# peabody124/PosePipeline

Measured on AMD Instinct MI355X. Metric: frames/sec (whole node), detect->2D->3D cascade on 1080p; MPJPE vs reference, higher is better.
Workload: dtype f32; eligible float32 convolutions are evaluated as 2-term float16 splits (22 significand bits under per-channel / per-sample power-of-two scales, 3 products per term) on the 16-bit matrix cores with float32 accumulation (float32-accurate at any input magnitude, not bit-identical: tests/test_gpu_spl

## Files before the change

posepipeline_amd/csrc/api_core.hip:

```cpp
#include <dlfcn.h>

#include <algorithm>
#include <memory>

#include "pp_internal.h"
#include "pp_amax.h"

#include <atomic>
extern std::atomic<int> g_decode_generic, g_split_gemm_epi;

static thread_local std::string g_last_error;

void pp_set_error(const char* fmt, ...) {
    char buf[1024];
    va_list ap;
    va_start(ap, fmt);
    vsnprintf(buf, sizeof(buf), fmt, ap);
    va_end(ap);
    g_last_error = buf;
}

namespace {
struct Roctx {
    int (*push)(const char*) = nullptr;
    int (*pop)() = nullptr;
    Roctx() {
        for (const char* lib : {"librocprofiler-sdk-roctx.so", "librocprofiler-sdk-roctx.so.1", "libroctx64.so", "libroctx64.so.4"}) {
            void* h = dlopen(lib, RTLD_LAZY | RTLD_LOCAL);
            if (!h) continue;
            push = reinterpret_cast<int (*)(const char*)>(dlsym(h, "roctxRangePushA"));
            pop = reinterpret_cast<int (*)()>(dlsym(h, "roctxRangePop"));
            if (push && pop) return;
            push = nullptr; pop = nullptr;
        }
    }
};
const Roctx& roctx() {
    static const Roctx r;
    return r;
}
}

void pp_range_push(const char* name) {
    if (roctx().push) (void)roctx().push(name);
}
void pp_range_pop() {
    if (roctx().pop) (void)roctx().pop();
}

int pp_ctx::ensure_scratch(size_t bytes) {
    if (bytes <= scratch_bytes) return PP_OK;
    if (scratch) {
        PP_HIP_CHECK(hipStreamSynchronize(stream));
        PP_HIP_CHECK(hipFree(scratch));
        scratch = nullptr;
        scratch_bytes = 0;
    }
    size_t want = std::max(bytes, size_t(1) << 20);
    PP_HIP_CHECK(hipMalloc(&scratch, want));
    scratch_bytes = want;
    return PP_OK;
}

extern "C" {

int pp_abi_version(void) { return PP_ABI_VERSION; }

int pp_debug_knob(const char* name, int value) {
    PP_REQUIRE(name && value >= -1 && value <= 1, "pp_debug_knob: name and a value in {-1, 0, 1}");
    if (!strcmp(name, "decode_generic")) g_decode_generic.store(value, std::memory_order_relaxed);
    else if (!strcmp(name, "split_gemm_epilogue")) g_split_gemm_epi.store(value, std::memory_order_relaxed);
    else {
        pp_set_error("pp_debug_knob: unknown knob '%s' (decode_generic, split_gemm_epilogue)", name);
        return PP_ERR_ARG;
    }
    return PP_OK;
}

const char* pp_last_error(void) { return g_last_error.c_str(); }

int pp_device_count(void) {
    int n = 0;
    if (hipGetDeviceCount(&n) != hipSuccess) {
        (void)hipGetLastError();
        return 0;
    }
    return n;
}

int pp_ctx_create(int device, pp_ctx** out) {
    PP_REQUIRE(out != nullptr, "pp_ctx_create: out is NULL");
    *out = nullptr;
    int n = 0;
    hipError_t e = hipGetDeviceCount(&n);
    if (e != hipSuccess || n <= 0) {
        (void)hipGetLastError();
        pp_set_error("pp_ctx_create: no HIP device visible (%s) -- this library has no CPU fallback",
                     e == hipSuccess ? "device count 0" : hipGetErrorString(e));
        return PP_ERR_HIP;
    }
    PP_REQUIRE(device >= 0 && device < n, "pp_ctx_create: device %d out of range [0,%d)", device, n);
    PP_HIP_CHECK(hipSetDevice(device));
    std::unique_ptr<pp_ctx> c(new pp_ctx());
    c->device = device;
    PP_HIP_CHECK(hipStreamCreateWithFlags(&c->stream, hipStreamNonBlocking));
    PP_HIP_CHECK(hipEventCreate(&c->ev_start));
// ... 143 lines not shown

struct pp_net {
    pp_ctx* ctx = nullptr;
    std::vector<pp_op> ops;
    std::vector<pp_buf> bufs;
    std::vector<size_t> buf_off;
    std::vector<size_t> buf_elems;
    float* weights = nullptr;
    size_t n_weights = 0;
    unsigned char* wsplit = nullptr;
    std::vector<long long> wsplit_off;
    int numerics = PP_NET_NUMERICS_EXACT;
    int split_f16 = 0;
    unsigned* amax = nullptr;
    std::vector<int> op_x_slot, op_y_slot, op_post_slot, slot_owner;
    std::vector<int> slot_first, slot_last;
    struct ExtAmax { int buf, slot, first_reader, last_reader; bool provided; };
    std::vector<ExtAmax> ext;
    float* arena = nullptr;
    size_t arena_floats = 0;
    int max_batch = 0;
    hipGraphExec_t graph_exec = nullptr;
    int graph_batch = 0;
    bool use_lanes = true;
    std::vector<hipStream_t> lanes;
    std::vector<int> op_lane;
    std::vector<std::vector<int>> op_waits;
    std::vector<char> op_needs_event;
    std::vector<hipEvent_t> op_done;
    hipEvent_t fork_ev = nullptr;
    std::vector<hipEvent_t> join_ev;
    std::vector<pp_vit_encoder*> vits;
    std::vector<pp_deconv_bf16*> deconvs;

    float* buf_ptr(int b) const { return arena + buf_off[b]; }
    unsigned* amax_slot(int slot) const { return slot >= 0 ? amax + (size_t)slot * max_batch : nullptr; }
};

static ConvArgs net_conv_args(pp_net* net, const pp_op& op, int batch);
static int net_make_lanes(pp_net* net, int n_lanes);

static void net_plan_amax(pp_net* net) {
    const int n = (int)net->ops.size(), nb = (int)net->bufs.size();
    net->op_x_slot.assign(n, -1);
    net->op_y_slot.assign(n, -1);
    net->op_post_slot.assign(n, -1);
    net->slot_owner.clear();
    net->ext.clear();
    if (net->numerics != PP_NET_NUMERICS_SPLIT || !net->split_f16) return;
    auto is_h = [&](int i) { return net->ops[i].type == PP_OP_CONV && net->wsplit_off[i] >= 0; };
    auto tracks = [&](int i) {
        const pp_op& op = net->ops[i];
        if (op.type == PP_OP_UPSAMPLE_ADD) return true;
        return op.type == PP_OP_CONV && pp_conv_tracks_amax(net_conv_args(net, op, 1), is_h(i));
    };
    {
        std::vector<char> written(nb, 0);
        for (int i = 0; i < n; ++i) {
            const pp_op& op = net->ops[i];
            if (is_h(i) && !written[op.in]) {
                pp_net::ExtAmax* e = nullptr;
                for (auto& x : net->ext)
                    if (x.buf == op.in) e = &x;
                if (!e) {
                    net->ext.push_back({op.in, (int)net->slot_owner.size(), i, i, false});
                    net->slot_owner.push_back(-1);
// ... 44 lines not shown
            for (int p : t.producers) net->op_y_slot[p] = t.slot;
        else
            net->op_post_slot[t.producers.back()] = t.slot;
    }
    for (const auto& r : readers) net->op_x_slot[r.first] = tensors[r.second].slot;
}

static int net_reset_amax(pp_net* net, int first, int last, int batch, hipStream_t s) {
    if (!net->amax) return PP_OK;
    int s0 = -1, s1 = -1;
    for (int k = 0; k < (int)net->slot_first.size(); ++k) {
        const int a = net->slot_first[k], b = net->slot_last[k];
        if (a < 0 || b < first || a >= last) continue;
        PP_REQUIRE(a >= first && b < last, "pp_net_run: op range [%d, %d) splits the producers (ops %d .. %d) of a tensor whose per-sample maxima are tracked",
                   first, last, a, b);
    }
    for (int k = 0; k < (int)net->slot_owner.size(); ++k)
        if (net->slot_owner[k] >= first && net->slot_owner[k] < last) {
            if (s0 < 0) s0 = k;
            s1 = k + 1;
        }
    if (s0 >= 0) PP_HIP_CHECK(hipMemsetAsync(net->amax_slot(s0), 0, (size_t)(s1 - s0) * net->max_batch * sizeof(unsigned), s));
    for (auto& e : net->ext) {
        if (e.last_reader < first || e.first_reader >= last) continue;
        if (e.provided) {
            e.provided = false;
            continue;
        }
        PP_HIP_CHECK(hipMemsetAsync(net->amax_slot(e.slot), 0, (size_t)batch * sizeof(unsigned), s));
        int rc = pp_launch_amax(net->buf_ptr(e.buf), batch, net->buf_elems[e.buf], net->amax_slot(e.slot), s);
        if (rc != PP_OK) return rc;
    }
    return PP_OK;
}

static void net_plan_lanes(pp_net* net, int n_lanes) {
    const int n = (int)net->ops.size(), nb = (int)net->bufs.size();
    net->op_lane.assign(n, 0);
    net->op_waits.assign(n, {});
    net->op_needs_event.assign(n, 0);
    std::vector<int> last_writer(nb, -1);
    std::vector<std::vector<int>> readers(nb);
    std::vector<int> lane_tail(n_lanes, -1);
    for (int i = 0; i < n; ++i) {
        const pp_op& op = net->ops[i];
        std::vector<int> deps;
        auto add = [&](int d) {
            if (d >= 0 && std::find(deps.begin(), deps.end(), d) == deps.end()) deps.push_back(d);
        };
        for (int b : {op.in, op.res1, op.res2, op.in2, op.in3})
            if (b >= 0) add(last_writer[b]);
        add(last_writer[op.out]);
        for (int r : readers[op.out]) add(r);
        int lane = -1, best = -1;
        for (int l = 0; l < n_lanes; ++l)
            if (lane_tail[l] >= 0 && lane_tail[l] > best && std::find(deps.begin(), deps.end(), lane_tail[l]) != deps.end()) {
                best = lane_tail[l];
                lane = l;
            }
        if (lane < 0) {
            lane = 0;
            for (int l = 1; l < n_lanes; ++l)
                if (lane_tail[l] < lane_tail[lane]) lane = l;
        }
        net->op_lane[i] = lane;
        for (int d : deps)
// ... 110 lines not shown
    a.y = net->buf_ptr(op.out);
    a.w = net->weights + op.w_off;
    a.bias = net->weights + op.b_off;
    a.res1 = op.res1 >= 0 ? net->buf_ptr(op.res1) : nullptr;
    a.res2 = op.res2 >= 0 ? net->buf_ptr(op.res2) : nullptr;
    a.N = batch; a.Hin = bi.h; a.Win = bi.w; a.Cin = op.cin;
    a.Hout = bo.h >> op.up_log2; a.Wout = bo.w >> op.up_log2;
    a.Cout = op.cout; a.CoutPad = (op.cout + 15) / 16 * 16;
    a.KH = op.kh; a.KW = op.kw; a.stride = op.stride; a.pad_h = op.pad_h; a.pad_w = op.pad_w;
    a.dil_h = op.dil_h; a.dil_w = op.dil_w;
    a.K = op.kh * op.kw * op.cin; a.Kpad = (a.K + 31) / 32 * 32;
    a.HWout = a.Hout * a.Wout; a.M = batch * a.HWout;
    a.relu = op.relu; a.up_log2 = op.up_log2; a.out_nchw = op.out_nchw;
    a.res1_shift = op.res1_shift; a.res1_off_w = op.res1_off_w;
    a.res1_H = op.res1 >= 0 ? net->bufs[op.res1].h : 0;
    a.res1_W = op.res1 >= 0 ? net->bufs[op.res1].w : 0;
    a.y_stride = bo.c; a.y_coff = op.out_c_off;
    a.x_pad = bi.pad; a.y_pad = bo.pad;
    a.r1_pad = op.res1 >= 0 ? net->bufs[op.res1].pad : 0;
    a.r2_pad = op.res2 >= 0 ? net->bufs[op.res2].pad : 0;
    const size_t idx = &op - net->ops.data();
    a.wsplit = (net->wsplit && idx < net->wsplit_off.size() && net->wsplit_off[idx] >= 0) ? net->wsplit + net->wsplit_off[idx] : nullptr;
    a.numerics = net->numerics;
    a.split_f16 = net->split_f16;
    if (idx < net->op_x_slot.size()) {
        a.x_amax = net->amax_slot(net->op_x_slot[idx]);
        a.y_amax = net->amax_slot(net->op_y_slot[idx]);
    }
    return a;
}

static int net_launch_op_body(pp_net* net, const pp_op& op, int batch, hipStream_t s);

static int net_launch_op(pp_net* net, const pp_op& op, int batch, hipStream_t s) {
    const size_t idx = &op - net->ops.data();
    int rc = net_launch_op_body(net, op, batch, s);
    if (rc == PP_OK && net->amax && net->op_post_slot[idx] >= 0)
        rc = pp_launch_amax(net->buf_ptr(op.out), batch, net->buf_elems[op.out], net->amax_slot(net->op_post_slot[idx]), s);
    return rc;
}

static int net_launch_op_body(pp_net* net, const pp_op& op, int batch, hipStream_t s) {
    const pp_buf& bi = net->bufs[op.in];
    const pp_buf& bo = net->bufs[op.out];
    if (op.type == PP_OP_CONV) {
        const ConvArgs a = net_conv_args(net, op, batch);
        return pp_launch_conv(a, s);
    } else if (op.type == PP_OP_MAXPOOL) {
        PoolArgs p{};
        p.x = net->buf_ptr(op.in); p.y = net->buf_ptr(op.out);
        p.N = batch; p.Hin = bi.h; p.Win = bi.w; p.C = op.cin; p.Hout = bo.h; p.Wout = bo.w;
        p.x_stride = bi.c; p.x_coff = op.in_c_off; p.y_stride = bo.c; p.y_coff = op.out_c_off;
        p.KH = op.kh; p.KW = op.kw; p.stride = op.stride; p.pad_h = op.pad_h; p.pad_w = op.pad_w;
        return pp_launch_maxpool(p, s);
    } else if (op.type == PP_OP_AVGPOOL) {
        return pp_launch_avgpool(net->buf_ptr(op.in), net->buf_ptr(op.out), batch, bi.h, bi.w, op.cin, op.kh, op.kw, op.stride, s);
    } else if (op.type == PP_OP_COPY) {
        PP_HIP_CHECK(hipMemcpyAsync(net->buf_ptr(op.out), net->buf_ptr(op.in),
                                    (size_t)batch * net->buf_elems[op.in] * sizeof(float),
                                    hipMemcpyDeviceToDevice, s));
        return PP_OK;
    } else if (op.type == PP_OP_DEPTH_TO_SPACE) {
        return pp_launch_depth_to_space(net->buf_ptr(op.in), net->buf_ptr(op.out), batch, bi.h, bi.w, op.cout, s);
    } else if (op.type == PP_OP_DECONV_BF16) {
        return pp_deconv_bf16_run(net->deconvs[&op - net->ops.data()], net->buf_ptr(op.in), net->buf_ptr(op.out), batch,
                                  op.relu == PP_RELU_LAST, s);
    } else if (op.type == PP_OP_UPSAMPLE_ADD) {
        return pp_launch_upsample_add(net->buf_ptr(op.in), op.res1 >= 0 ? net->buf_ptr(op.res1) : nullptr,
// ... 94 lines not shown
        if (op.type != PP_OP_VIT_ENCODER) continue;
        const pp_buf& bi = net->bufs[op.in];
        int rc = pp_vit_encoder_create(net->weights + op.w_off, bi.h * bi.w, op.cin, op.kh, op.kw, op.cin * op.stride,
                                       max_batch, ctx->stream, &net->vits[i]);
        if (rc != PP_OK) {
            pp_net_destroy(net.release());
            return rc;
        }
    }
    net->wsplit_off.assign(n_ops, -1);
    if (net->numerics == PP_NET_NUMERICS_SPLIT) {
        size_t bytes = 0;
        for (int i = 0; i < n_ops; ++i) {
            if (net->ops[i].type != PP_OP_CONV) continue;
            const ConvArgs a = net_conv_args(net.get(), net->ops[i], 1);
            if (!pp_conv_split_eligible(a)) continue;
            net->wsplit_off[i] = (long long)bytes;
            bytes += (pp_conv_split_bytes(a) + 255) / 256 * 256;
        }
        net_plan_amax(net.get());
        if (!net->slot_owner.empty()) {
            const size_t ab = net->slot_owner.size() * (size_t)max_batch * sizeof(unsigned);
            PP_HIP_CHECK(hipMalloc((void**)&net->amax, ab));
            PP_HIP_CHECK(hipMemsetAsync(net->amax, 0, ab, ctx->stream));
        }
        if (bytes) {
            PP_HIP_CHECK(hipMalloc((void**)&net->wsplit, bytes));
            for (int i = 0; i < n_ops; ++i) {
                if (net->wsplit_off[i] < 0) continue;
                const ConvArgs a = net_conv_args(net.get(), net->ops[i], 1);
                int rc = pp_conv_split_weights(a, net->wsplit + net->wsplit_off[i], ctx->stream);
                if (rc != PP_OK) return rc;
            }
        }
    }
    PP_HIP_CHECK(hipStreamSynchronize(ctx->stream));
    for (int i = 0; i < n_ops; ++i)
        if (net->ops[i].type == PP_OP_CONV) {
            int rc = pp_conv_prepare(net_conv_args(net.get(), net->ops[i], 1));
            if (rc != PP_OK) return rc;
        }
    const char* env_lanes = getenv("POSEPIPE_NET_LANES");
    const int n_lanes = env_lanes ? atoi(env_lanes) : 4;
    int rc_l = net_make_lanes(net.get(), n_lanes);
    if (rc_l != PP_OK) return rc_l;
    *out = net.release();
    return PP_OK;
}

static int net_make_lanes(pp_net* net, int n_lanes) {
    for (auto l : net->lanes) (void)hipStreamDestroy(l);
    net->lanes.clear();
    for (auto e : net->op_done)
        if (e) (void)hipEventDestroy(e);
    net->op_done.clear();
    for (auto e : net->join_ev)
        if (e) (void)hipEventDestroy(e);
    net->join_ev.clear();
    if (net->fork_ev) (void)hipEventDestroy(net->fork_ev);
    net->fork_ev = nullptr;
    const int n_ops = (int)net->ops.size();
    if (n_lanes > 1 && n_ops >= 8) {
        net_plan_lanes(net, n_lanes);
        net->lanes.resize(n_lanes);
        for (auto& l : net->lanes) PP_HIP_CHECK(hipStreamCreateWithFlags(&l, hipStreamNonBlocking));
        net->op_done.assign(n_ops, nullptr);
// ... 46 lines not shown
    for (auto* d : net->deconvs) pp_deconv_bf16_destroy(d);
    if (net->weights) (void)hipFree(net->weights);
    if (net->wsplit) (void)hipFree(net->wsplit);
    if (net->amax) (void)hipFree(net->amax);
    if (net->arena) (void)hipFree(net->arena);
    delete net;
}

int pp_net_buffer(pp_net* net, int buf, void** dptr, size_t* bytes_per_sample) {
    PP_REQUIRE(net && buf >= 0 && buf < (int)net->bufs.size(), "pp_net_buffer: bad buffer id");
    PP_REQUIRE(net->bufs[buf].pad == 0, "pp_net_buffer: buffer %d has a zero halo (conv-internal layout); expose dense buffers only", buf);
    if (dptr) *dptr = net->buf_ptr(buf);
    if (bytes_per_sample) *bytes_per_sample = net->buf_elems[buf] * sizeof(float);
    return PP_OK;
}

int pp_net_run(pp_net* net, int batch, int first_op, int last_op) {
    PP_REQUIRE(net, "pp_net_run: net is NULL");
    PP_REQUIRE(batch > 0 && batch <= net->max_batch, "pp_net_run: batch %d not in (0,%d]", batch, net->max_batch);
    if (last_op < 0) last_op = (int)net->ops.size();
    PP_REQUIRE(first_op >= 0 && last_op <= (int)net->ops.size() && first_op <= last_op, "pp_net_run: bad op range");
    if (net->graph_exec && batch == net->graph_batch && first_op == 0 && last_op == (int)net->ops.size()) {
        PP_HIP_CHECK(hipGraphLaunch(net->graph_exec, net->ctx->stream));
        return PP_OK;
    }
    hipStream_t main = net->ctx->stream;
    PpRange range("pp_net_run");
    {
        int rc = net_reset_amax(net, first_op, last_op, batch, main);
        if (rc != PP_OK) return rc;
    }
    if (net->lanes.empty() || !net->use_lanes || last_op - first_op < 8) {
        for (int i = first_op; i < last_op; ++i) {
            int rc = net_launch_op(net, net->ops[i], batch, main);
            if (rc != PP_OK) return rc;
        }
        return PP_OK;
    }
    PP_HIP_CHECK(hipEventRecord(net->fork_ev, main));
    for (hipStream_t l : net->lanes) PP_HIP_CHECK(hipStreamWaitEvent(l, net->fork_ev, 0));
    for (int i = first_op; i < last_op; ++i) {
        hipStream_t s = net->lanes[net->op_lane[i]];
        for (int d : net->op_waits[i])
            if (d >= first_op) PP_HIP_CHECK(hipStreamWaitEvent(s, net->op_done[d], 0));
        int rc = net_launch_op(net, net->ops[i], batch, s);
        if (rc != PP_OK) return rc;
        if (net->op_needs_event[i]) PP_HIP_CHECK(hipEventRecord(net->op_done[i], s));
    }
    for (size_t l = 0; l < net->lanes.size(); ++l) {
        PP_HIP_CHECK(hipEventRecord(net->join_ev[l], net->lanes[l]));
        PP_HIP_CHECK(hipStreamWaitEvent(main, net->join_ev[l], 0));
    }
    return PP_OK;
}

int pp_net_vit_timing(pp_net* net, int enable, float* ms3, int* n_gemm) {
    PP_REQUIRE(net, "pp_net_vit_timing: net is NULL");
    for (auto* v : net->vits) {
        if (!v) continue;
        if (ms3) {
            PP_HIP_CHECK(hipStreamSynchronize(net->ctx->stream));
            int rc = pp_vit_encoder_get_timing(v, ms3, n_gemm);
            if (rc != PP_OK) return rc;
        }
        pp_vit_encoder_set_timing(v, enable);
        return PP_OK;
    }
    pp_set_error("pp_net_vit_timing: the program has no PP_OP_VIT_ENCODER");
    return PP_ERR_STATE;
}

int pp_net_set_lane_count(pp_net* net, int n_lanes) {
    PP_REQUIRE(net && n_lanes >= 1 && n_lanes <= 16, "pp_net_set_lane_count: net is NULL or n_lanes not in [1, 16]");
    PP_HIP_CHECK(hipStreamSynchronize(net->ctx->stream));
    for (auto l : net->lanes) PP_HIP_CHECK(hipStreamSynchronize(l));
    if (net->graph_exec) {
        PP_HIP_CHECK(hipGraphExecDestroy(net->graph_exec));
        net->graph_exec = nullptr;
    }
    return net_make_lanes(net, n_lanes);
}

int pp_net_set_lanes(pp_net* net, int enable) {
    PP_REQUIRE(net, "pp_net_set_lanes: net is NULL");
    PP_HIP_CHECK(hipStreamSynchronize(net->ctx->stream));
    net->use_lanes = enable != 0;
    return PP_OK;
}

int pp_net_capture(pp_net* net, int batch) {
    PP_REQUIRE(net, "pp_net_capture: net is NULL");
    PP_REQUIRE(batch > 0 && batch <= net->max_batch, "pp_net_capture: bad batch");
    if (net->graph_exec) {
        PP_HIP_CHECK(hipGraphExecDestroy(net->graph_exec));
        net->graph_exec = nullptr;
    }
    hipStream_t s = net->ctx->stream;
    PP_HIP_CHECK(hipStreamSynchronize(s));
    hipGraph_t graph = nullptr;
    PP_HIP_CHECK(hipStreamBeginCapture(s, hipStreamCaptureModeThreadLocal));
    int rc = net_reset_amax(net, 0, (int)net->ops.size(), batch, s);
    for (size_t i = 0; i < net->ops.size() && rc == PP_OK; ++i) rc = net_launch_op(net, net->ops[i], batch, s);
    hipError_t e = hipStreamEndCapture(s, &graph);
    if (rc != PP_OK) {
        if (graph) (void)hipGraphDestroy(graph);
        return rc;
    }
    PP_HIP_CHECK(e);
    PP_HIP_CHECK(hipGraphInstantiate(&net->graph_exec, graph, nullptr, nullptr, 0));
    PP_HIP_CHECK(hipGraphDestroy(graph));
    net->graph_batch = batch;
    return PP_OK;
}

int pp_net_forward(pp_net* net, int batch, int in_buf, const float* in, int out_buf, float* out, int mem) {
    PP_REQUIRE(net && in && out, "pp_net_forward: NULL argument");
    PP_REQUIRE(in_buf >= 0 && in_buf < (int)net->bufs.size() && out_buf >= 0 && out_buf < (int)net->bufs.size(),
               "pp_net_forward: bad buffer id");
    PP_REQUIRE(batch > 0 && batch <= net->max_batch, "pp_net_forward: batch %d not in (0,%d]", batch, net->max_batch);
    PP_REQUIRE(net->bufs[in_buf].pad == 0 && net->bufs[out_buf].pad == 0, "pp_net_forward: input / output buffers must be dense (pad 0)");
    hipStream_t s = net->ctx->stream;
    const hipMemcpyKind kin = mem == PP_MEM_HOST ? hipMemcpyHostToDevice : hipMemcpyDeviceToDevice;
    const hipMemcpyKind kout = mem == PP_MEM_HOST ? hipMemcpyDeviceToHost : hipMemcpyDeviceToDevice;
    PP_HIP_CHECK(hipMemcpyAsync(net->buf_ptr(in_buf), in, (size_t)batch * net->buf_elems[in_buf] * sizeof(float), kin, s));
    for (auto& e : net->ext)
        if (e.buf == in_buf) e.provided = false;
    int rc = pp_net_run(net, batch, 0, (int)net->ops.size());
    if (rc != PP_OK) return rc;
    PP_HIP_CHECK(hipMemcpyAsync(out, net->buf_ptr(out_buf), (size_t)batch * net->buf_elems[out_buf] * sizeof(float), kout, s));
    PP_HIP_CHECK(hipStreamSynchronize(s));
    return PP_OK;
}

int pp_net_profile(pp_net* net, int batch, float* ms_per_op) {
    PP_REQUIRE(net, "pp_net_profile: net is NULL");
    PP_REQUIRE(batch > 0 && batch <= net->max_batch, "pp_net_profile: bad batch");
    hipStream_t s = net->ctx->stream;
    const size_t n = net->ops.size();
    std::vector<hipEvent_t> ev(n + 1);
    for (auto& e : ev) PP_HIP_CHECK(hipEventCreate(&e));
    int rc = net_reset_amax(net, 0, (int)n, batch, s);
    PP_HIP_CHECK(hipEventRecord(ev[0], s));
    for (size_t i = 0; i < n && rc == PP_OK; ++i) {
        rc = net_launch_op(net, net->ops[i], batch, s);
        if (rc == PP_OK && hipEventRecord(ev[i + 1], s) != hipSuccess) rc = PP_ERR_HIP;
    }
    if (rc == PP_OK && hipStreamSynchronize(s) != hipSuccess) rc = PP_ERR_HIP;
    if (rc == PP_OK && ms_per_op) {
        for (size_t i = 0; i < n; ++i) {
            float ms = 0.f;
            (void)hipEventElapsedTime(&ms, ev[i], ev[i + 1]);
            ms_per_op[i] = ms;
        }
    }
    for (auto& e : ev) (void)hipEventDestroy(e);
    return rc;
}

int pp_conv2d(pp_ctx* ctx, const pp_op* op, int n, int hin, int win, const float* x, const float* w,
              const float* bias, const float* res1, const float* res2, float* y, int res1_h, int res1_w,
              int mem) {
    PP_REQUIRE(ctx && op && x && w && bias && y, "pp_conv2d: NULL argument");
    PP_REQUIRE(op->type == PP_OP_CONV, "pp_conv2d: op is not a conv");
    PP_REQUIRE(n > 0 && hin > 0 && win > 0, "pp_conv2d: empty input");
    ConvArgs a{};
    a.N = n; a.Hin = hin; a.Win = win; a.Cin = op->cin;
    a.Hout = pp_conv_out_dim(hin + (op->pad_end & 1), op->kh, op->stride, op->pad_h, op->dil_h) - ((op->pad_end >> 2) & 1);
    a.Wout = pp_conv_out_dim(win + ((op->pad_end >> 1) & 1), op->kw, op->stride, op->pad_w, op->dil_w) - ((op->pad_end >> 3) & 1);
    PP_REQUIRE(a.Hout > 0 && a.Wout > 0, "pp_conv2d: empty output");
    a.Cout = op->cout; a.CoutPad = (op->cout + 15) / 16 * 16;
    a.KH = op->kh; a.KW = op->kw; a.stride = op->stride; a.pad_h = op->pad_h; a.pad_w = op->pad_w;
    a.dil_h = op->dil_h; a.dil_w = op->dil_w;
    a.K = op->kh * op->kw * op->cin; a.Kpad = (a.K + 31) / 32 * 32;
    a.HWout = a.Hout * a.Wout; a.M = n * a.HWout;
    a.relu = op->relu; a.up_log2 = op->up_log2; a.out_nchw = op->out_nchw;
    a.res1_shift = op->res1_shift; a.res1_off_w = op->res1_off_w;
    const int Ho2 = a.Hout << op->up_log2, Wo2 = a.Wout << op->up_log2;
// ... 41 lines not shown
```

posepipeline_amd/csrc/conv_split.hip:

```cpp
#include <algorithm>
#include <atomic>
#include <map>
#include <mutex>
#include <type_traits>
#include <vector>
#include <cstring>
#include <cstdio>

#include "pp_internal.h"
#include "pp_amax.h"

#ifndef PP_SPLIT_ABLATE
#define PP_SPLIT_ABLATE 0
#endif

typedef __attribute__((ext_vector_type(8))) __bf16 bf16x8;
typedef __attribute__((ext_vector_type(8))) _Float16 f16x8;
typedef __attribute__((ext_vector_type(16))) float f32x16;

std::atomic<int> g_split_gemm_epi{-1};

namespace {


// ... 1063 lines not shown
            }
    }
    float ymax[SB];
#pragma unroll
    for (int sb = 0; sb < SB; ++sb) {
        ymax[sb] = 0.f;
#pragma unroll
        for (int cb = 0; cb < CB; ++cb) {
            float4 v = rv[sb][cb];
            if (a.relu == PP_RELU_LAST) { v.x = fmaxf(v.x, 0.f); v.y = fmaxf(v.y, 0.f); v.z = fmaxf(v.z, 0.f); v.w = fmaxf(v.w, 0.f); }
            if (ook[sb] && cok[cb]) {
                *reinterpret_cast<float4*>(a.y + ypix[sb] * a.Cout + cos[cb]) = v;
                ymax[sb] = fmaxf(ymax[sb], pp_abs4max(v));
            }
        }
    }
    if (a.y_amax) {
        int wg_first = n, wg_last = n;
        if (a.mode != MODE_TILE) {
            const unsigned last = (unsigned)min((long long)s0 + 255, a.S - 1);
            wg_first = (int)pp_udiv(min(s0, last), a.dv_per);
            wg_last = (int)pp_udiv(last, a.dv_per);
        }
        pp_amax_commit_wg<4, SB>(a.y_amax, onn, ymax, wg_first, wg_last, reinterpret_cast<float*>(smem));
    }
    PP_TL_MARK(3);
#ifdef PP_SPLIT_TIMELINE
    asm volatile("s_waitcnt vmcnt(0)" ::: "memory");
    PP_TL_MARK(7);
#endif
    PP_TL_FLUSH();
}

__device__ __forceinline__ float channel_scale(float cmax) {
    if (!(cmax > 0.f) || !(cmax < 3.0e38f)) return 1.f;
    int e;
    (void)frexpf(cmax, &e);
    return ldexpf(1.f, 15 - e);
}
__device__ __forceinline__ void split_weight_h(float v, float c, unsigned short& q0, unsigned short& q1, unsigned short& q2) {
    const float vs = v * c;
    const _Float16 g0 = (_Float16)vs;
    const float r = vs - (float)g0;
    const _Float16 g1 = (_Float16)r;
    q0 = __builtin_bit_cast(unsigned short, g0);
    q1 = __builtin_bit_cast(unsigned short, g1);
    q2 = 0;
}
__global__ __launch_bounds__(64) void weight_channel_max_kernel(const float* w, int kchunks, int CoutPad, int nout, float* cmax, float* inv_scale) {
    const int cout = blockIdx.x, lane = threadIdx.x;
    float m = 0.f;
    if (cout < CoutPad)
        for (int c = lane >> 5; c < kchunks; c += 2) m = fmaxf(m, fabsf(w[((size_t)c * CoutPad + cout) * 32 + (lane & 31)]));
#pragma unroll
    for (int o = 32; o > 0; o >>= 1) m = fmaxf(m, __shfl_xor(m, o));
    if (lane == 0 && cout < nout) {
        cmax[cout] = m;
        inv_scale[cout] = 1.f / channel_scale(m);
    }
}

template <bool H>
__global__ __launch_bounds__(256) void split_weights48_kernel(const float* w, uint4* out, int Cin, int CoutPad, int ncb16, size_t total, const float* cmax) {
    const size_t i = blockIdx.x * (size_t)256 + threadIdx.x;
    if (i >= total) return;
    const int lane = (int)(i & 63);
// ... 889 lines not shown
        hipError_t es = hipGetLastError();
        if (es != hipSuccess) {
            pp_set_error("split_weights_stem7 launch failed: %s", hipGetErrorString(es));
            return PP_ERR_HIP;
        }
        return PP_OK;
    }
    if (split_c48(a)) {
        const size_t total48 = (size_t)(cin / 16) * 5 * split_ncb16(a) * 64;
        if (a.split_f16)
            hipLaunchKernelGGL(split_weights48_kernel<true>, dim3((unsigned)((total48 + 255) / 256)), dim3(256), 0, stream, a.w, (uint4*)out, cin,
                               a.CoutPad, split_ncb16(a), total48, cmax);
        else
        hipLaunchKernelGGL(split_weights48_kernel<false>, dim3((unsigned)((total48 + 255) / 256)), dim3(256), 0, stream, a.w, (uint4*)out, cin,
                           a.CoutPad, split_ncb16(a), total48, cmax);
        hipError_t e48 = hipGetLastError();
        if (e48 != hipSuccess) {
            pp_set_error("split_weights48 launch failed: %s", hipGetErrorString(e48));
            return PP_ERR_HIP;
        }
        return PP_OK;
    }
    const size_t total = (size_t)(cin / 16) * taps * ncb * 64;
    if (a.split_f16)
        hipLaunchKernelGGL(split_weights_kernel<true>, dim3((unsigned)((total + 255) / 256)), dim3(256), 0, stream, a.w, (uint4*)out, cin,
                           taps, a.CoutPad, ncb, total, cmax);
    else
    hipLaunchKernelGGL(split_weights_kernel<false>, dim3((unsigned)((total + 255) / 256)), dim3(256), 0, stream, a.w, (uint4*)out, cin,
                       taps, a.CoutPad, ncb, total, cmax);
    hipError_t e = hipGetLastError();
    if (e != hipSuccess) {
        pp_set_error("split_weights launch failed: %s", hipGetErrorString(e));
        return PP_ERR_HIP;
    }
    return PP_OK;
}

__global__ __launch_bounds__(256) void amax_kernel(const float4* x, size_t quads, unsigned per, unsigned* amax) {
    const unsigned n = blockIdx.x / per, part = blockIdx.x - n * per;
    const float4* xs = x + (size_t)n * quads;
    float m = 0.f;
    for (size_t i = (size_t)part * 256 + threadIdx.x; i < quads; i += (size_t)per * 256) m = fmaxf(m, pp_abs4max(xs[i]));
    __shared__ float red[16];
    const int im[1] = {(int)n};
    const float mm[1] = {m};
    pp_amax_commit_wg<4, 1>(amax, im, mm, (int)n, (int)n, red);
}

int pp_launch_amax(const float* x, int n, size_t elems, unsigned* amax, hipStream_t stream) {
    if (n <= 0 || elems == 0) return PP_OK;
    if (elems % 4 != 0) {
        pp_set_error("amax: %zu floats per sample (a multiple of 4 is required)", elems);
        return PP_ERR_ARG;
    }
    const size_t quads = elems / 4;
    const unsigned per = (unsigned)std::min<size_t>(std::max<size_t>((quads + 1023) / 1024, 1), std::max<size_t>(2048 / (size_t)n, 1));
    hipLaunchKernelGGL(amax_kernel, dim3(per * (unsigned)n), dim3(256), 0, stream, (const float4*)x, quads, per, amax);
    hipError_t e = hipGetLastError();
    if (e != hipSuccess) {
        pp_set_error("amax launch failed: %s", hipGetErrorString(e));
        return PP_ERR_HIP;
    }
    return PP_OK;
}

#ifdef PP_SPLIT_TIMELINE
// ... 362 lines not shown
```

posepipeline_amd/csrc/pp_internal.h:

```cpp
#pragma once
#include <hip/hip_runtime.h>
#include <cstdarg>
#include <cstdio>
#include <cstring>
#include <string>
#include <vector>
#include <mutex>

#include "posepipe_hip.h"

void pp_set_error(const char* fmt, ...);

#define PP_HIP_CHECK(expr)                                                              \
    do {                                                                                \
        hipError_t _e = (expr);                                                         \
        if (_e != hipSuccess) {                                                         \
            pp_set_error("%s failed: %s (%s:%d)", #expr, hipGetErrorString(_e), __FILE__, \
                         __LINE__);                                                     \
            return PP_ERR_HIP;                                                          \
        }                                                                               \
    } while (0)

#define PP_REQUIRE(cond, ...)            \
    do {                                 \
// ... 60 lines not shown
    ~PpStages() { next(nullptr); }
};

struct ConvArgs {
    const float* x;
    const float* w;
    const float* bias;
    const float* res1;
    const float* res2;
    float* y;
    int N, Hin, Win, Cin, Hout, Wout, Cout, CoutPad;
    int KH, KW, stride, pad_h, pad_w, dil_h, dil_w;
    int K, Kpad, M, HWout;
    unsigned div_hw_m, div_hw_s1, div_hw_s2, div_w_m, div_w_s1, div_w_s2;
    unsigned div_c_m, div_c_s1, div_c_s2, div_kw_m, div_kw_s1, div_kw_s2;
    int xcd_remap;
    unsigned x_bytes;
    int relu, up_log2, out_nchw;
    int res1_shift, res1_off_w, res1_H, res1_W;
    int y_stride, y_coff;
    const uint2* tap_table;
    int x_pad, y_pad, r1_pad, r2_pad;
    int no_bounds;
    const void* wsplit;
    int numerics;
    int split_f16;
    const unsigned* x_amax;
    unsigned* y_amax;
};
bool pp_conv_split_eligible(const ConvArgs& a);
size_t pp_conv_split_bytes(const ConvArgs& a);
int pp_conv_split_weights(const ConvArgs& a, void* out, hipStream_t stream);
int pp_launch_conv_split(const ConvArgs& a, hipStream_t stream);
bool pp_conv_tracks_amax(const ConvArgs& a, bool split);
bool pp_conv_split_enabled();
bool pp_conv_split_f16_default();
int pp_conv_prepare(const ConvArgs& a);
int pp_conv_out_dim(int in, int k, int stride, int pad, int dil);
int pp_launch_conv(const ConvArgs& a, hipStream_t stream);
int pp_launch_conv_p3(const ConvArgs& a, int ct, int pt, hipStream_t stream, bool fake_addresses = false);

struct PoolArgs {
    const float* x;
    float* y;
    int N, Hin, Win, C, Hout, Wout, KH, KW, stride, pad_h, pad_w;
    int x_stride, x_coff, y_stride, y_coff;
};
int pp_launch_maxpool(const PoolArgs& a, hipStream_t stream);
int pp_launch_avgpool(const float* x, float* y, int n, int hin, int win, int c, int kh, int kw, int stride, hipStream_t stream);

struct GemmArgs {
    const void* A;
    const void* B;
    const float* bias;
    const float* res;
    void* C;
    int M, N, K;
    int act;
    int out_bf16;
    int res_mod;
    int group_m;
    int qkv_tokens, qkv_hd;
};
int pp_launch_gemm_bf16(const GemmArgs& a, hipStream_t stream);
int pp_gemm_bf16_prepare();
struct pp_deconv_bf16;
// ... 41 lines not shown
```

Measured before the change: 616.3.

## Fuse consecutive 48-channel 3x3 split-f16 convs of basic residual blocks into one kernel

```diff
diff --git a/posepipeline_amd/csrc/api_core.hip b/posepipeline_amd/csrc/api_core.hip
--- a/posepipeline_amd/csrc/api_core.hip
+++ b/posepipeline_amd/csrc/api_core.hip
@@ -8,6 +8,7 @@
 
 #include <atomic>
 extern std::atomic<int> g_decode_generic, g_split_gemm_epi;
+static std::atomic<int> g_fuse_basic{-1};
 
 static thread_local std::string g_last_error;
 
@@ -70,8 +71,9 @@
     PP_REQUIRE(name && value >= -1 && value <= 1, "pp_debug_knob: name and a value in {-1, 0, 1}");
     if (!strcmp(name, "decode_generic")) g_decode_generic.store(value, std::memory_order_relaxed);
     else if (!strcmp(name, "split_gemm_epilogue")) g_split_gemm_epi.store(value, std::memory_order_relaxed);
+    else if (!strcmp(name, "fuse_basic")) g_fuse_basic.store(value, std::memory_order_relaxed);
     else {
-        pp_set_error("pp_debug_knob: unknown knob '%s' (decode_generic, split_gemm_epilogue)", name);
+        pp_set_error("pp_debug_knob: unknown knob '%s' (decode_generic, split_gemm_epilogue, fuse_basic)", name);
         return PP_ERR_ARG;
     }
     return PP_OK;
@@ -281,6 +283,7 @@
     std::vector<hipEvent_t> join_ev;
     std::vector<pp_vit_encoder*> vits;
     std::vector<pp_deconv_bf16*> deconvs;
+    std::vector<int> pair_next;
 
     float* buf_ptr(int b) const { return arena + buf_off[b]; }
     unsigned* amax_slot(int slot) const { return slot >= 0 ? amax + (size_t)slot * max_batch : nullptr; }
@@ -391,6 +394,32 @@
         if (rc != PP_OK) return rc;
     }
     return PP_OK;
+}
+
+static void net_plan_pairs(pp_net* net) {
+    const int n = (int)net->ops.size();
+    net->pair_next.assign(n, -1);
+    static const int env = [] { const char* e = getenv("POSEPIPE_FUSE_BASIC"); return e ? atoi(e) : 1; }();
+    const int knob = g_fuse_basic.load(std::memory_order_relaxed);
+    if (!(knob >= 0 ? knob : env) || !net->split_f16) return;
+    bool any = false;
+    for (int i = 0; i + 1 < n; ++i) {
+        const pp_op &o1 = net->ops[i], &o2 = net->ops[i + 1];
+        if (o1.type != PP_OP_CONV || o2.type != PP_OP_CONV || net->wsplit_off[i] < 0 || net->wsplit_off[i + 1] < 0) continue;
+        if (net->bufs[o1.out].pad < 1 || o2.in != o1.out || o1.in == o1.out || net->op_post_slot[i] >= 0) continue;
+        if (i > 0 && net->pair_next[i - 1] >= 0) continue;
+        bool only = o2.res1 != o1.out && o2.res2 != o1.out && o2.out != o1.out && o2.out != o1.in;
+        for (int k = i + 2; k < n && only; ++k) {
+            const pp_op& o = net->ops[k];
+            for (int b : {o.in, o.res1, o.res2, o.in2, o.in3})
+                if (b == o1.out) only = false;
+            if (o.out == o1.out) break;
+        }
+        if (!only || !pp_conv_split_pair_eligible(net_conv_args(net, o1, 1), net_conv_args(net, o2, 1))) continue;
+        net->pair_next[i] = i + 1;
+        any = true;
+    }
+    if (!any) net->pair_next.clear();
 }
 
 static void net_plan_lanes(pp_net* net, int n_lanes) {
@@ -567,8 +596,15 @@
 
 static int net_launch_op_body(pp_net* net, const pp_op& op, int batch, hipStream_t s);
 
-static int net_launch_op(pp_net* net, const pp_op& op, int batch, hipStream_t s) {
-    const size_t idx = &op - net->ops.data();
+static int net_launch_op(pp_net* net, const pp_op& op, int batch, hipStream_t s, int first, int last) {
+    const int idx = (int)(&op - net->ops.data());
+    if (!net->pair_next.empty()) {
+        const int j = net->pair_next[idx];
+        if (j >= 0 && j < last) return PP_OK;
+        const int i = idx - 1;
+        if (i >= first && net->pair_next[i] == idx)
+            return pp_launch_conv_split_pair(net_conv_args(net, net->ops[i], batch), net_conv_args(net, op, batch), s);
+    }
     int rc = net_launch_op_body(net, op, batch, s);
     if (rc == PP_OK && net->amax && net->op_post_slot[idx] >= 0)
         rc = pp_launch_amax(net->buf_ptr(op.out), batch, net->buf_elems[op.out], net->amax_slot(net->op_post_slot[idx]), s);
@@ -729,6 +765,7 @@
                 int rc = pp_conv_split_weights(a, net->wsplit + net->wsplit_off[i], ctx->stream);
                 if (rc != PP_OK) return rc;
             }
+            net_plan_pairs(net.get());
         }
     }
     PP_HIP_CHECK(hipStreamSynchronize(ctx->stream));
@@ -841,7 +878,7 @@
     }
     if (net->lanes.empty() || !net->use_lanes || last_op - first_op < 8) {
         for (int i = first_op; i < last_op; ++i) {
-            int rc = net_launch_op(net, net->ops[i], batch, main);
+            int rc = net_launch_op(net, net->ops[i], batch, main, first_op, last_op);
             if (rc != PP_OK) return rc;
         }
         return PP_OK;
@@ -852,7 +889,7 @@
         hipStream_t s = net->lanes[net->op_lane[i]];
         for (int d : net->op_waits[i])
             if (d >= first_op) PP_HIP_CHECK(hipStreamWaitEvent(s, net->op_done[d], 0));
-        int rc = net_launch_op(net, net->ops[i], batch, s);
+        int rc = net_launch_op(net, net->ops[i], batch, s, first_op, last_op);
         if (rc != PP_OK) return rc;
         if (net->op_needs_event[i]) PP_HIP_CHECK(hipEventRecord(net->op_done[i], s));
     }
@@ -909,7 +946,7 @@
     hipGraph_t graph = nullptr;
     PP_HIP_CHECK(hipStreamBeginCapture(s, hipStreamCaptureModeThreadLocal));
     int rc = net_reset_amax(net, 0, (int)net->ops.size(), batch, s);
-    for (size_t i = 0; i < net->ops.size() && rc == PP_OK; ++i) rc = net_launch_op(net, net->ops[i], batch, s);
+    for (size_t i = 0; i < net->ops.size() && rc == PP_OK; ++i) rc = net_launch_op(net, net->ops[i], batch, s, 0, (int)net->ops.size());
     hipError_t e = hipStreamEndCapture(s, &graph);
     if (rc != PP_OK) {
         if (graph) (void)hipGraphDestroy(graph);
@@ -951,7 +988,7 @@
     int rc = net_reset_amax(net, 0, (int)n, batch, s);
     PP_HIP_CHECK(hipEventRecord(ev[0], s));
     for (size_t i = 0; i < n && rc == PP_OK; ++i) {
-        rc = net_launch_op(net, net->ops[i], batch, s);
+        rc = net_launch_op(net, net->ops[i], batch, s, 0, (int)n);
         if (rc == PP_OK && hipEventRecord(ev[i + 1], s) != hipSuccess) rc = PP_ERR_HIP;
     }
     if (rc == PP_OK && hipStreamSynchronize(s) != hipSuccess) rc = PP_ERR_HIP;
diff --git a/posepipeline_amd/csrc/conv_split.hip b/posepipeline_amd/csrc/conv_split.hip
--- a/posepipeline_amd/csrc/conv_split.hip
+++ b/posepipeline_amd/csrc/conv_split.hip
@@ -1119,6 +1119,276 @@
     PP_TL_FLUSH();
 }
 
+struct PairArgs {
+    const float* x;
+    const uint4* w1;
+    const uint4* w2;
+    const float* wscale1;
+    const float* wscale2;
+    const float* b1;
+    const float* b2;
+    float* y;
+    const unsigned* x_amax;
+    unsigned* y_amax;
+    int H, W, xp_h, xp_w, y_pad;
+    int tiles_x, tiles_y;
+    unsigned x_bytes;
+    unsigned dv_tx[2], dv_ty[2];
+};
+
+constexpr int pair_pad8(int n) { return n + ((12 - n % 8) % 8); }
+
+template <int TW>
+__global__ __launch_bounds__(256, 2) void conv_split48_pair_kernel(PairArgs a) {
+    constexpr int NT = 256, NPAIR = 5, CB = 3, NCH = 3, SB1 = 6, SB2 = 4, WPL = 2, NST = NCH * NPAIR;
+    constexpr int TH = 256 / TW, XW = TW + 4, NPx = (TH + 4) * XW, NPxp = pair_pad8(NPx), MW = TW + 2, NM = (TH + 2) * MW, NMp = pair_pad8(NM);
+    constexpr int NSLOT = (NPx + NT / 4 - 1) / (NT / 4);
+    static_assert(NM <= 4 * SB1 * 16 && NSLOT <= 7, "tile too large for the register budget");
+    extern __shared__ __attribute__((aligned(16))) unsigned char smem[];
+    const int tid = threadIdx.x;
+    const int lane = tid & 63;
+    const int wave = tid >> 6;
+    const unsigned L = blockIdx.x;
+    const unsigned Lq = pp_udiv(L, a.dv_tx);
+    const int tx = (int)(L - Lq * (unsigned)a.tiles_x);
+    const int n = (int)pp_udiv(Lq, a.dv_ty);
+    const int ty = (int)(Lq - (unsigned)n * (unsigned)a.tiles_y);
+    const int x0 = tx * TW, y0 = ty * TH;
+    constexpr int xplane = 2 * NPxp * 16, xbuf = 2 * xplane;
+    constexpr int mplane = 2 * NMp * 16, mchunk = 2 * mplane;
+    unsigned goff[NSLOT];
+#pragma unroll
+    for (int j = 0; j < NSLOT; ++j) {
+        const int p = (tid >> 2) + (NT / 4) * j;
+        const int pr = p / XW, pc = p - pr * XW;
+        const int iy = y0 - 2 + pr, ix = x0 - 2 + pc;
+        goff[j] = 0xffffffffu;
+        if (p < NPx && (unsigned)iy < (unsigned)a.H && (unsigned)ix < (unsigned)a.W)
+            goff[j] = (unsigned)(((n * a.xp_h + iy) * a.xp_w + ix) * 48) * 4u + (unsigned)(tid & 3) * 16u;
+    }
+    const __amdgpu_buffer_rsrc_t xrsrc = __builtin_amdgcn_make_buffer_rsrc((void*)a.x, 0, (int)a.x_bytes, 0x00020000);
+    float4 xr[NSLOT];
+    auto load_patch = [&](int c) {
+#pragma unroll
+        for (int j = 0; j < NSLOT; ++j) {
+            const unsigned off = goff[j] == 0xffffffffu ? 0xffffffffu : goff[j] + (unsigned)c * 64u;
+            xr[j] = __builtin_bit_cast(float4, __builtin_amdgcn_raw_buffer_load_b128(xrsrc, (int)off, 0, 0));
+        }
+    };
+    const int woff0 = ((((tid & 3) >> 1) * NPxp + (tid >> 2)) * 16 + (tid & 1) * 8);
+    auto store_patch = [&](int buf, float sx) {
+#pragma unroll
+        for (int j = 0; j < NSLOT; ++j) {
+            uint2 p0, p1;
+            split4h(xr[j], sx, p0, p1);
+            if ((tid >> 2) + (NT / 4) * j >= NPx) continue;
+            unsigned char* d = smem + buf * xbuf + woff0 + (NT / 4) * 16 * j;
+            *reinterpret_cast<uint2*>(d) = p0;
+            *reinterpret_cast<uint2*>(d + xplane) = p1;
+        }
+    };
+    constexpr int WSTEP = CB * WPL * 64;
+    uint4 wf[2][CB][WPL];
+    auto load_w = [&](int gs, uint4 (&dst)[CB][WPL]) {
+        const uint4* wp = (gs < NST ? a.w1 + (size_t)gs * WSTEP : a.w2 + (size_t)(gs - NST) * WSTEP) + lane;
+#pragma unroll
+        for (int cb = 0; cb < CB; ++cb)
+#pragma unroll
+            for (int pl = 0; pl < WPL; ++pl) dst[cb][pl] = wp[(cb * WPL + pl) * 64];
+    };
+    load_patch(0);
+    load_w(0, wf[0]);
+    const unsigned xam = a.x_amax[n];
+    __builtin_amdgcn_sched_barrier(0);
+    const int khalf = (lane >> 4) & 1;
+    int aof1[SB1];
+#pragma unroll
+    for (int sb = 0; sb < SB1; ++sb) {
+        const int i0 = (wave * SB1 + sb) * 16 + (lane & 15), i = i0 < NM ? i0 : 0;
+        const int mr = i / MW, mc = i - mr * MW;
+        aof1[sb] = (khalf * NPxp + mr * XW + mc) * 16;
+    }
+    const int hi = lane >> 5;
+    auto tofs = [&](int q, int pitch) {
+        const int t0 = 2 * q, t1 = min(2 * q + 1, 8);
+        return hi ? ((t1 / 3) * pitch + (t1 % 3)) * 16 : ((t0 / 3) * pitch + (t0 % 3)) * 16;
+    };
+    uint4 xf[2][2];
+    auto load_x = [&](const unsigned char* pbuf, int pb, int off, int sb) {
+        xf[sb & 1][0] = *reinterpret_cast<const uint4*>(pbuf + off);
+        xf[sb & 1][1] = *reinterpret_cast<const uint4*>(pbuf + pb + off);
+    };
+    auto mma = [&](f32x4 (&acc)[CB], const uint4 (&wc)[CB][WPL], int sb) {
+        constexpr int WI[3] = {1, 0, 0}, XI[3] = {0, 1, 0};
+#pragma unroll
+        for (int p = 0; p < 3; ++p)
+#pragma unroll
+            for (int cb = 0; cb < CB; ++cb)
+                acc[cb] = __builtin_amdgcn_mfma_f32_16x16x32_f16(__builtin_bit_cast(f16x8, wc[cb][WI[p]]), __builtin_bit_cast(f16x8, xf[sb & 1][XI[p]]),
+                                                                 acc[cb], 0, 0, 0);
+    };
+    const float sx = pp_act_scale(xam), xinv = pp_act_unscale(xam);
+    store_patch(0, sx);
+    load_patch(1);
+    __syncthreads();
+    f32x4 acc1[SB1][CB];
+#pragma unroll
+    for (int sb = 0; sb < SB1; ++sb)
+#pragma unroll
+        for (int cb = 0; cb < CB; ++cb) acc1[sb][cb] = f32x4{0.f, 0.f, 0.f, 0.f};
+    load_x(smem, xplane, aof1[0] + tofs(0, XW), 0);
+#pragma unroll
+    for (int c = 0; c < NCH; ++c) {
+        const unsigned char* pbuf = smem + (c & 1) * xbuf;
+#pragma unroll
+        for (int q = 0; q < NPAIR; ++q) {
+            const int gs = c * NPAIR + q, cur = gs & 1;
+            load_w(gs + 1, wf[cur ^ 1]);
+            __builtin_amdgcn_sched_barrier(0);
+#pragma unroll
+            for (int sb = 0; sb < SB1; ++sb) {
+                if (sb == SB1 - 1 && q == NPAIR / 2 && c + 1 < NCH) store_patch((c + 1) & 1, sx);
+                if (sb + 1 < SB1) load_x(pbuf, xplane, aof1[sb + 1] + tofs(q, XW), sb + 1);
+                else if (q + 1 < NPAIR) load_x(pbuf, xplane, aof1[0] + tofs(q + 1, XW), 0);
+                __builtin_amdgcn_sched_barrier(0);
+                mma(acc1[sb], wf[cur], sb);
+                __builtin_amdgcn_sched_barrier(0);
+            }
+        }
+        __syncthreads();
+        if (c + 1 < NCH) load_x(smem + ((c + 1) & 1) * xbuf, xplane, aof1[0] + tofs(0, XW), 0);
+        if (c + 2 < NCH) load_patch(c + 2);
+    }
+    constexpr int RED = (2 * xbuf > NCH * mchunk ? 2 * xbuf : NCH * mchunk);
+    const int g = lane >> 4;
+    float minv;
+    {
+        float4 b4[CB], sc4[CB];
+#pragma unroll
+        for (int cb = 0; cb < CB; ++cb) {
+            b4[cb] = *reinterpret_cast<const float4*>(a.b1 + cb * 16 + 4 * g);
+            sc4[cb] = *reinterpret_cast<const float4*>(a.wscale1 + cb * 16 + 4 * g);
+        }
+        float m = 0.f;
+#pragma unroll
+        for (int sb = 0; sb < SB1; ++sb) {
+            const int i = (wave * SB1 + sb) * 16 + (lane & 15);
+            const int mr = i / MW, mc = i - mr * MW;
+            const int iy = y0 - 1 + mr, ix = x0 - 1 + mc;
+            const bool inside = i < NM && (unsigned)iy < (unsigned)a.H && (unsigned)ix < (unsigned)a.W;
+#pragma unroll
+            for (int cb = 0; cb < CB; ++cb) {
+                const f32x4 cc = acc1[sb][cb];
+                f32x4 v = {__builtin_fmaf(cc[0], sc4[cb].x * xinv, b4[cb].x), __builtin_fmaf(cc[1], sc4[cb].y * xinv, b4[cb].y),
+                           __builtin_fmaf(cc[2], sc4[cb].z * xinv, b4[cb].z), __builtin_fmaf(cc[3], sc4[cb].w * xinv, b4[cb].w)};
+#pragma unroll
+                for (int e = 0; e < 4; ++e) v[e] = inside ? fmaxf(v[e], 0.f) : 0.f;
+                acc1[sb][cb] = v;
+                m = fmaxf(m, fmaxf(fmaxf(v[0], v[1]), fmaxf(v[2], v[3])));
+            }
+        }
+        m = pp_wave_max(m);
+        float* red = reinterpret_cast<float*>(smem + RED);
+        if (lane == 0) red[wave] = m;
+        __syncthreads();
+        const unsigned mam = __float_as_uint(fmaxf(fmaxf(red[0], red[1]), fmaxf(red[2], red[3])));
+        const float smid = pp_act_scale(mam);
+        minv = pp_act_unscale(mam);
+#pragma unroll
+        for (int sb = 0; sb < SB1; ++sb) {
+            const int i = (wave * SB1 + sb) * 16 + (lane & 15);
+#pragma unroll
+            for (int cb = 0; cb < CB; ++cb) {
+                const f32x4 v4 = acc1[sb][cb];
+                const float4 v = make_float4(v4[0], v4[1], v4[2], v4[3]);
+                uint2 p0, p1;
+                split4h(v, smid, p0, p1);
+                if (i < NM) {
+                    unsigned char* d = smem + cb * mchunk + ((g >> 1) * NMp + i) * 16 + (g & 1) * 8;
+                    *reinterpret_cast<uint2*>(d) = p0;
+                    *reinterpret_cast<uint2*>(d + mplane) = p1;
+                }
+            }
+        }
+    }
+    __syncthreads();
+    int aof2[SB2];
+#pragma unroll
+    for (int sb = 0; sb < SB2; ++sb) {
+        const int j = (wave * SB2 + sb) * 16 + (lane & 15);
+        const int orow = j / TW, ocol = j - orow * TW;
+        aof2[sb] = (khalf * NMp + orow * MW + ocol) * 16;
+    }
+    f32x4 acc2[SB2][CB];
+#pragma unroll
+    for (int sb = 0; sb < SB2; ++sb)
+#pragma unroll
+        for (int cb = 0; cb < CB; ++cb) acc2[sb][cb] = f32x4{0.f, 0.f, 0.f, 0.f};
+    load_x(smem, mplane, aof2[0] + tofs(0, MW), 0);
+#pragma unroll
+    for (int c = 0; c < NCH; ++c) {
+        const unsigned char* pbuf = smem + c * mchunk;
+#pragma unroll
+        for (int q = 0; q < NPAIR; ++q) {
+            const int gs = NST + c * NPAIR + q, cur = gs & 1;
+            if (gs + 1 < 2 * NST) load_w(gs + 1, wf[cur ^ 1]);
+            __builtin_amdgcn_sched_barrier(0);
+#pragma unroll
+            for (int sb = 0; sb < SB2; ++sb) {
+                if (sb + 1 < SB2) load_x(pbuf, mplane, aof2[sb + 1] + tofs(q, MW), sb + 1);
+                else if (q + 1 < NPAIR) load_x(pbuf, mplane, aof2[0] + tofs(q + 1, MW), 0);
+                else if (c + 1 < NCH) load_x(pbuf + mchunk, mplane, aof2[0] + tofs(0, MW), 0);
+                __builtin_amdgcn_sched_barrier(0);
+                mma(acc2[sb], wf[cur], sb);
+                __builtin_amdgcn_sched_barrier(0);
+            }
+        }
+    }
+    float4 b4[CB], sc4[CB];
+#pragma unroll
+    for (int cb = 0; cb < CB; ++cb) {
+        b4[cb] = *reinterpret_cast<const float4*>(a.b2 + cb * 16 + 4 * g);
+        sc4[cb] = *reinterpret_cast<const float4*>(a.wscale2 + cb * 16 + 4 * g);
+    }
+    size_t xpix[SB2], ypix[SB2];
+    bool ook[SB2];
+#pragma unroll
+    for (int sb = 0; sb < SB2; ++sb) {
+        const int j = (wave * SB2 + sb) * 16 + (lane & 15);
+        const int orow = j / TW, ocol = j - orow * TW;
+        const int oy = y0 + orow, ox = x0 + ocol;
+        ook[sb] = oy < a.H && ox < a.W;
+        const int y_ = ook[sb] ? oy : 0, x_ = ook[sb] ? ox : 0;
+        xpix[sb] = ((size_t)n * a.xp_h + y_) * a.xp_w + x_;
+        ypix[sb] = ((size_t)n * (a.H + a.y_pad) + y_) * (a.W + a.y_pad) + x_;
+    }
+    float4 rv[SB2][CB];
+#pragma unroll
+    for (int sb = 0; sb < SB2; ++sb)
+#pragma unroll
+        for (int cb = 0; cb < CB; ++cb) rv[sb][cb] = *reinterpret_cast<const float4*>(a.x + xpix[sb] * 48 + cb * 16 + 4 * g);
+    float ymax[SB2];
+    int onn[SB2];
+#pragma unroll
+    for (int sb = 0; sb < SB2; ++sb) {
+        ymax[sb] = 0.f;
+        onn[sb] = n;
+#pragma unroll
+        for (int cb = 0; cb < CB; ++cb) {
+            const f32x4 cc = acc2[sb][cb];
+            float4 v = make_float4(__builtin_fmaf(cc[0], sc4[cb].x * minv, b4[cb].x), __builtin_fmaf(cc[1], sc4[cb].y * minv, b4[cb].y),
+                                   __builtin_fmaf(cc[2], sc4[cb].z * minv, b4[cb].z), __builtin_fmaf(cc[3], sc4[cb].w * minv, b4[cb].w));
+            v.x += rv[sb][cb].x; v.y += rv[sb][cb].y; v.z += rv[sb][cb].z; v.w += rv[sb][cb].w;
+            v.x = fmaxf(v.x, 0.f); v.y = fmaxf(v.y, 0.f); v.z = fmaxf(v.z, 0.f); v.w = fmaxf(v.w, 0.f);
+            if (ook[sb]) {
+                *reinterpret_cast<float4*>(a.y + ypix[sb] * 48 + cb * 16 + 4 * g) = v;
+                ymax[sb] = fmaxf(ymax[sb], pp_abs4max(v));
+            }
+        }
+    }
+    if (a.y_amax) pp_amax_commit_wg<4, SB2>(a.y_amax, onn, ymax, n, n, reinterpret_cast<float*>(smem));
+}
+
 __device__ __forceinline__ float channel_scale(float cmax) {
     if (!(cmax > 0.f) || !(cmax < 3.0e38f)) return 1.f;
     int e;
@@ -2074,6 +2344,66 @@
     if (e != hipSuccess) {
         pp_set_error("split_weights launch failed: %s", hipGetErrorString(e));
         return PP_ERR_HIP;
+    }
+    return PP_OK;
+}
+
+static int pair_tile_w(int H, int W) {
+    const long t8 = (long)((H + 31) / 32) * ((W + 7) / 8), t16 = (long)((H + 15) / 16) * ((W + 15) / 16);
+    return t8 <= t16 ? 8 : 16;
+}
+
+bool pp_conv_split_pair_eligible(const ConvArgs& a1, const ConvArgs& a2) {
+    auto c48 = [](const ConvArgs& a) {
+        return a.split_f16 && a.wsplit && split_c48(a) && a.Cin == 48 && a.Cout == 48 && a.KH == 3 && a.KW == 3 && a.stride == 1 &&
+               a.pad_h == 1 && a.pad_w == 1 && a.dil_h == 1 && a.dil_w == 1 && a.Hin == a.Hout && a.Win == a.Wout &&
+               (a.y_stride == 0 || a.y_stride == 48) && a.y_coff == 0;
+    };
+    return c48(a1) && c48(a2) && a1.relu == PP_RELU_LAST && !a1.res1 && !a1.res2 && a2.relu == PP_RELU_LAST && a2.x == a1.y &&
+           a2.res1 == a1.x && a2.res1_shift == 0 && a2.r1_pad == a1.x_pad && !a2.res2 && a1.Hin == a2.Hin && a1.Win == a2.Win;
+}
+
+int pp_launch_conv_split_pair(const ConvArgs& a1, const ConvArgs& a2, hipStream_t stream) {
+    if (!a1.x_amax) {
+        pp_set_error("conv_split pair: the fp16 form needs the per-sample maximum of its input (ConvArgs::x_amax)");
+        return PP_ERR_STATE;
+    }
+    PairArgs s{};
+    s.x = a1.x; s.y = a2.y;
+    s.w1 = (const uint4*)a1.wsplit; s.w2 = (const uint4*)a2.wsplit;
+    s.wscale1 = reinterpret_cast<const float*>(static_cast<const unsigned char*>(a1.wsplit) + split_frag_bytes(a1, true));
+    s.wscale2 = reinterpret_cast<const float*>(static_cast<const unsigned char*>(a2.wsplit) + split_frag_bytes(a2, true));
+    s.b1 = a1.bias; s.b2 = a2.bias;
+    s.H = a1.Hout; s.W = a1.Wout; s.xp_h = a1.Hin + a1.x_pad; s.xp_w = a1.Win + a1.x_pad; s.y_pad = a2.y_pad;
+    const int TW = pair_tile_w(s.H, s.W), TH = 256 / TW;
+    s.tiles_x = (s.W + TW - 1) / TW;
+    s.tiles_y = (s.H + TH - 1) / TH;
+    make_magic((unsigned)s.tiles_x, s.dv_tx);
+    make_magic((unsigned)s.tiles_y, s.dv_ty);
+    const size_t lds = std::max<size_t>((size_t)2 * 2 * 2 * pair_pad8((TH + 4) * (TW + 4)) * 16, (size_t)3 * 2 * 2 * pair_pad8((TH + 2) * (TW + 2)) * 16) + 16;
+    static PpPerDeviceOnce once;
+    once.run([] {
+        (void)hipFuncSetAttribute((const void*)conv_split48_pair_kernel<8>, hipFuncAttributeMaxDynamicSharedMemorySize, 80 * 1024);
+        (void)hipFuncSetAttribute((const void*)conv_split48_pair_kernel<16>, hipFuncAttributeMaxDynamicSharedMemorySize, 80 * 1024);
+    });
+    const size_t img = (size_t)s.xp_h * s.xp_w * 48 * sizeof(float), yimg = (size_t)(s.H + s.y_pad) * (s.W + s.y_pad) * 48;
+    const int per = (int)std::max<size_t>(1, 0xfffffff0u / img);
+    for (int n0 = 0; n0 < a1.N; n0 += per) {
+        PairArgs p = s;
+        const int nb = std::min(per, a1.N - n0);
+        p.x = s.x + (size_t)n0 * (img / sizeof(float));
+        p.y = s.y + (size_t)n0 * yimg;
+        p.x_amax = a1.x_amax + n0;
+        p.y_amax = a2.y_amax ? a2.y_amax + n0 : nullptr;
+        p.x_bytes = (unsigned)(nb * img);
+        const dim3 grid((unsigned)(s.tiles_x * s.tiles_y * nb));
+        if (TW == 8) hipLaunchKernelGGL(conv_split48_pair_kernel<8>, grid, dim3(256), lds, stream, p);
+        else hipLaunchKernelGGL(conv_split48_pair_kernel<16>, grid, dim3(256), lds, stream, p);
+        hipError_t e = hipGetLastError();
+        if (e != hipSuccess) {
+            pp_set_error("conv_split48_pair launch failed: %s", hipGetErrorString(e));
+            return PP_ERR_HIP;
+        }
     }
     return PP_OK;
 }
diff --git a/posepipeline_amd/csrc/pp_internal.h b/posepipeline_amd/csrc/pp_internal.h
--- a/posepipeline_amd/csrc/pp_internal.h
+++ b/posepipeline_amd/csrc/pp_internal.h
@@ -116,6 +116,8 @@
 size_t pp_conv_split_bytes(const ConvArgs& a);
 int pp_conv_split_weights(const ConvArgs& a, void* out, hipStream_t stream);
 int pp_launch_conv_split(const ConvArgs& a, hipStream_t stream);
+bool pp_conv_split_pair_eligible(const ConvArgs& a1, const ConvArgs& a2);
+int pp_launch_conv_split_pair(const ConvArgs& a1, const ConvArgs& a2, hipStream_t stream);
 bool pp_conv_tracks_amax(const ConvArgs& a, bool split);
 bool pp_conv_split_enabled();
 bool pp_conv_split_f16_default();
```

New measurement: 620.7 (median of 6 runs). About the same (+0.7%).
